# gwall-ceres/HighRes-net

Measured on AMD Instinct MI355X. Metric: SR frames/sec (384x384 out) at B=32, n_views=32, higher is better.
Workload: dtype bf16

## Files before the change

### highres-net_amd/hrnet_hip/csrc/conv3x3_v6_impl.h

```cpp
#pragma once
#include <type_traits>
#include "conv3x3.h"

#ifndef V6_ABL
#define V6_ABL 0
#endif
#ifndef V6_ST_AUX
#define V6_ST_AUX 2
#endif
#ifndef V6_RES_NT
#define V6_RES_NT 1
#endif
#ifndef V6_BAL
#define V6_BAL 4
#endif

#ifdef V6_STAMP
extern __device__ unsigned long long hrn_v6_stamps[256 * 8 * 24];
#define V6_ST(i) do { unsigned long long t_; asm volatile("s_memtime %0\n\ts_waitcnt lgkmcnt(0)" : "=s"(t_) :: "memory"); if (stamp_on) st[i] = t_; } while (0)
#else
#define V6_ST(i) do {} while (0)
#endif

namespace {

constexpr int T6_H = 16, T6_W = 32;
constexpr int HW6 = T6_W + 2;
constexpr int NPIX6 = (T6_H + 2) * HW6;
constexpr int N_IN6 = (NPIX6 * 64 + 1023) / 1024;
constexpr int IN_BYTES6 = N_IN6 * 1024;
constexpr unsigned OOB6 = 0x80000000u;

template <int COUT, bool X3 = false> struct G6 {
    static constexpr int NCB = COUT / 16;
    static constexpr int NQ = NCB / 2;
    static constexpr int TAP_BYTES = COUT * 64;
    static constexpr int WST = 3 * TAP_BYTES;
    static constexpr int W_PIECES = WST / 1024;
    static constexpr int OFF_IN = 2 * WST;
    static constexpr int OFF_BIAS = OFF_IN + 2 * IN_BYTES6;
    static constexpr int ROW = COUT * 2;
    static constexpr int LB = NCB * 2;
    static constexpr int OFF_FIFO = OFF_BIAS + 512;
    static constexpr int FIFO_WAVE = (LB == 16 && !X3) ? 4096 : 0;
    static constexpr int OFF_HOFF = OFF_FIFO + 8 * FIFO_WAVE;
    static constexpr int LDS_BYTES = OFF_HOFF + (X3 ? 8 * 5 * 256 : 0);
};

typedef __attribute__((address_space(3))) void* lds_ptr6;

template <int N> __device__ __forceinline__ void wait_vm6() {
    static_assert(N >= 0 && N <= 63, "vmcnt");
    asm volatile("s_waitcnt vmcnt(%0)" :: "n"(N) : "memory");
}
__device__ __forceinline__ void wait_vm6_rt(int n) {
    switch (n) {
        case 1: wait_vm6<1>(); break;
        case 2: wait_vm6<2>(); break;
        case 3: wait_vm6<3>(); break;
        case 4: wait_vm6<4>(); break;
        case 5: wait_vm6<5>(); break;
        case 6: wait_vm6<6>(); break;
        case 7: wait_vm6<7>(); break;
        case 8: wait_vm6<8>(); break;
        case 9: wait_vm6<9>(); break;
        default: wait_vm6<0>(); break;
    }
}
__device__ __forceinline__ void barrier6() {
    asm volatile("s_waitcnt lgkmcnt(0)" ::: "memory");
    __builtin_amdgcn_s_barrier();
    asm volatile("" ::: "memory");
}
__device__ __forceinline__ int swz6(int row) { return ((row >> 2) & 1) << 1; }

template <int N, int I = 0, class F> __device__ __forceinline__ void static_for6(F&& f) {
    if constexpr (I < N) { f(std::integral_constant<int, I>{}); static_for6<N, I + 1>(f); }
}

template <int CIN, int COUT, int RESM, bool PAIR, bool X3>
__global__ __launch_bounds__(512, 2) void conv3x3_v6_kernel(const ConvParams p) {
    typedef G6<COUT, X3> GEO;
    static_assert(CIN == 128 || (CIN == 64 && !PAIR), "CIN");
    constexpr int NCH = CIN / 32;
    constexpr int NCC = X3 ? 3 * NCH : NCH;
    constexpr int NCB = GEO::NCB, NQ = GEO::NQ, NSTEP = 3 * NQ, WST = GEO::WST, TAP_BYTES = GEO::TAP_BYTES;
    constexpr int OFF_IN = GEO::OFF_IN, ROW = GEO::ROW, LB = GEO::LB;
    typedef typename std::conditional<LB == 16, u32x4, u32x2>::type lane_row_t;
    constexpr bool RES = RESM != 0;
    constexpr int BAL = COUT == 128 ? V6_BAL : 0;
    extern __shared__ __attribute__((aligned(16))) unsigned char smem[];
    float* bias_lds = (float*)(smem + GEO::OFF_BIAS);
    if constexpr (X3) {
        if (p.only_if_nonpos && p.only_if_nonpos[0] > 0.f) return;
    }

    const int tid = threadIdx.x;
    const int lane = tid & 63;
    const int w = __builtin_amdgcn_readfirstlane(tid >> 6);
    const int c15 = lane & 15, q = lane >> 4;
    const int H = p.H, W = p.W;
    const unsigned hw = (unsigned)(H * W);
    const unsigned tiles_x = (W + T6_W - 1) / T6_W;
    const unsigned tiles_y = (H + T6_H - 1) / T6_H;
    const unsigned tiles = tiles_x * tiles_y;
    const unsigned total = tiles * (unsigned)p.M;
    const unsigned G = gridDim.x;
    const unsigned bid = blockIdx.x;
    const unsigned slot0 = (G & 7) == 0 ? (bid & 7) * (G >> 3) + (bid >> 3) : bid;
    if (slot0 >= total) return;
    const int ntl = (int)((total - slot0 + G - 1) / G);
    unsigned cur_m = slot0 / tiles, cur_t = slot0 - cur_m * tiles;
    const unsigned step_m = G / tiles, step_t = G - step_m * tiles;
    constexpr bool in_pair = PAIR;
    constexpr unsigned in_pitch = in_pair ? 128u : (unsigned)(CIN * 2);
    const size_t src_lo = X3 ? (in_pair ? p.stack_lo : p.in_lo) : 0;
    const unsigned char* const src0 = (const unsigned char*)(in_pair ? p.stack : p.in);
    const unsigned img_bytes = hw * in_pitch;

    auto in_bases = [&](unsigned m, size_t& a, size_t& b) __attribute__((always_inline)) {
        if (in_pair) {
            const unsigned bb = m / (unsigned)p.pair_h, i = m - bb * (unsigned)p.pair_h;
            a = ((size_t)bb * p.pair_vs + i) * hw * 128;
            b = ((size_t)bb * p.pair_vs + (p.pair_last - i)) * hw * 128;
        } else {
            a = b = (size_t)m * hw * in_pitch;
        }
    };
    unsigned hoff[5];
    auto tile_offsets = [&](unsigned t) __attribute__((always_inline)) {
        const int ty = t / tiles_x;
        const int y0 = ty * T6_H, x0 = (t - ty * tiles_x) * T6_W;
        int lq = lane;
        asm volatile("" : "+v"(lq));
#pragma unroll
        for (int jj = 0; jj < 5; ++jj) {
            const int pix = (w + 8 * jj) * 16 + (lq >> 2);
            const int lc = (lq & 3) ^ swz6(pix);
            const int py = pix / HW6, px = pix - py * HW6;
            const int gy = y0 - 1 + py, gx = x0 - 1 + px;
            const bool ok = pix < NPIX6 && (unsigned)gy < (unsigned)H && (unsigned)gx < (unsigned)W;
            const unsigned ho = ok ? (unsigned)(gy * W + gx) * in_pitch + (unsigned)(lc * 16) : OOB6;
            if constexpr (X3) *(unsigned*)(smem + GEO::OFF_HOFF + (w * 5 + jj) * 256 + lq * 4) = ho;
            else hoff[jj] = ho;
        }
    };
    auto dma_halo_v = [&](__amdgpu_buffer_rsrc_t rs, int c, int buf, int jj, unsigned voff) __attribute__((always_inline)) {
        const int j = w + 8 * jj;
        if (j < N_IN6) {
            const unsigned soff = in_pair ? (unsigned)((c & 1) * 64) : (unsigned)(c * 64);
            if (!(V6_ABL & 4)) __builtin_amdgcn_raw_ptr_buffer_load_lds(rs, (lds_ptr6)(smem + OFF_IN + buf * IN_BYTES6 + j * 1024), 16, voff, soff, 0, 0);
        }
    };
    auto hoff_lds = [&](int jj) __attribute__((always_inline)) -> unsigned {
        return *(const unsigned*)(smem + GEO::OFF_HOFF + (w * 5 + jj) * 256 + lane * 4);
    };
    auto dma_halo = [&](__amdgpu_buffer_rsrc_t rs, int c, int buf, int jj) __attribute__((always_inline)) {
        if constexpr (X3) dma_halo_v(rs, c, buf, jj, hoff_lds(jj));
        else dma_halo_v(rs, c, buf, jj, hoff[jj]);
    };
    constexpr unsigned W_PLANE = 9u * CIN * COUT * 2u;
    const __amdgpu_buffer_rsrc_t rs_w = __builtin_amdgcn_make_buffer_rsrc((void*)p.wpk, 0, (int)(W_PLANE * (X3 ? 2 : 1)), 0x00020000);
    const unsigned w_lane_off = (unsigned)((lane >> 2) * (NCB * 128) + (((lane & 3) ^ swz6(lane >> 2)) << 4));
    auto dma_w = [&](int c, int tg, int slot_, int t3, unsigned plane_off) __attribute__((always_inline)) {
        const int qq = w + 8 * t3;
        if (qq < GEO::W_PIECES) {
            const int kx = qq / NCB, jb = qq - kx * NCB;
            const unsigned soff = plane_off + (unsigned)(((c >> 1) * 9 + tg * 3 + kx) * (COUT * 128) + (c & 1) * 64 + jb * 128);
            if (!(V6_ABL & 4)) __builtin_amdgcn_raw_ptr_buffer_load_lds(rs_w, (lds_ptr6)(smem + slot_ * WST + kx * TAP_BYTES + jb * 1024), 16, w_lane_off, soff, 0, 0);
        }
    };
    constexpr int NW3 = (GEO::W_PIECES + 7) / 8;
    const int n_in = w < (N_IN6 & 7) ? (N_IN6 >> 3) + 1 : (N_IN6 >> 3);

    const float act_slope = p.slope ? p.slope[0] : 1.f;
    const float act_pick = act_slope <= 1.f ? __builtin_inff() : -__builtin_inff();

    const unsigned lds0 = (unsigned)(__UINTPTR_TYPE__)(__attribute__((address_space(3))) unsigned char*)smem;
    const unsigned a_off = lds0 + (unsigned)(c15 * 64 + ((q ^ swz6(c15)) << 4));
    unsigned baddr[4][3];
#pragma unroll
    for (int j = 0; j < 4; ++j)
#pragma unroll
        for (int kx = 0; kx < 3; ++kx) {
            const int pix = (2 * w + j) * HW6 + c15 + kx;
            baddr[j][kx] = lds0 + (unsigned)OFF_IN + (unsigned)(pix << 6) + ((unsigned)(q << 4) ^ (unsigned)((pix & 4) << 3));
        }

    f32x4 acc[NCB][4];
#ifdef V6_STAMP
    unsigned long long st[24];
#pragma unroll
    for (int i = 0; i < 24; ++i) st[i] = 0;
    bool stamp_on = false;
#endif

    if (tid < COUT) bias_lds[tid] = p.bias[tid];
    size_t inA, inB;
    in_bases(cur_m, inA, inB);
    tile_offsets(cur_t);
    {
        const __amdgpu_buffer_rsrc_t rs = __builtin_amdgcn_make_buffer_rsrc((void*)(src0 + inA), 0, (int)img_bytes, 0x00020000);
#pragma unroll
        for (int t3 = 0; t3 < NW3; ++t3) dma_w(0, 0, 0, t3, 0u);
#pragma unroll
        for (int jj = 0; jj < 5; ++jj) dma_halo(rs, 0, 0, jj);
    }
    wait_vm6<0>();
    barrier6();

    for (int tl = 0; tl < ntl; ++tl) {
        const bool more_tiles = tl + 1 < ntl;
#ifdef V6_STAMP
        stamp_on = false;
        if (RESM == 2 && !PAIR && ntl >= 32 && tl == 1) { stamp_on = true; V6_ST(20); }
        if (RESM == 2 && !PAIR && ntl >= 32 && tl == 2) { stamp_on = true; V6_ST(21); stamp_on = false; }
#endif
        unsigned nxt_t = cur_t + step_t, nxt_m = cur_m + step_m;
        if (nxt_t >= tiles) { nxt_t -= tiles; ++nxt_m; }
        size_t nxA = inA, nxB = inB;
        if (more_tiles) in_bases(nxt_m, nxA, nxB);
#pragma unroll
        for (int cb4 = 0; cb4 < NCB; cb4 += 4) {
            const f32x4 b = *(const f32x4*)(bias_lds + NCB * c15 + cb4);
#pragma unroll
            for (int e = 0; e < 4; ++e)
#pragma unroll
                for (int pxb = 0; pxb < 4; ++pxb) acc[cb4 + e][pxb] = f32x4{b[e], b[e], b[e], b[e]};
        }
        const int ty_ = cur_t / tiles_x;
        const int y0 = ty_ * T6_H, x0 = (cur_t - ty_ * tiles_x) * T6_W;
        const unsigned char *resA = nullptr, *resB = nullptr;
        unsigned char* outp;
        float res_alpha = 1.f;
        {
            size_t oimg = cur_m;
            if (p.out_h > 0) {
                const unsigned ob = cur_m / (unsigned)p.out_h, oi = cur_m - ob * (unsigned)p.out_h;
                oimg = (size_t)ob * p.out_vs + oi;
                if (RESM == 3) {
                    resA = resB = (const unsigned char*)p.res + ((size_t)ob * p.res_vs + oi) * hw * 128;
                    if (p.alphas) res_alpha = p.alphas[(size_t)ob * p.alpha_vs + (p.pair_last - oi)];
                }
            }
            if (RESM == 2) {
                const unsigned bb = cur_m / (unsigned)p.pair_h, i = cur_m - bb * (unsigned)p.pair_h;
                resA = (const unsigned char*)p.stack + ((size_t)bb * p.pair_vs + i) * hw * 128;
                resB = (const unsigned char*)p.stack + ((size_t)bb * p.pair_vs + (p.pair_last - i)) * hw * 128;
            }
            if (RESM == 1) resA = resB = (const unsigned char*)p.res + (size_t)cur_m * hw * ROW;
            outp = (unsigned char*)p.out + oimg * hw * ROW;
        }
        auto res_src = [&](int r, int j) __attribute__((always_inline)) -> const unsigned char* {
            int lq = lane;
            asm volatile("" : "+v"(lq));
            const int c15r = lq & 15, qr = lq >> 4;
            const int gy = y0 + 2 * w + (r >> 1), gyc = gy < H ? gy : H - 1;
            const int gx = x0 + 16 * (r & 1) + 4 * qr + j, gxc = gx < W ? gx : W - 1;
            const unsigned char* view = (RESM == 2 && c15r >= 8) ? resB : resA;
            constexpr int RPITCH = RESM == 1 ? ROW : 128;
            if (V6_ABL & 64) return resA + ((unsigned)(((gyc * W + gxc) & 511) * RPITCH) + (RESM == 2 ? (unsigned)((c15r & 7) * 16) : (unsigned)(c15r * LB)));
            return view + ((unsigned)((gyc * W + gxc) * RPITCH) + (RESM == 2 ? (unsigned)((c15r & 7) * 16) : (unsigned)(c15r * LB)));
        };
        constexpr bool FIFO = RES && LB == 16 && !X3;
        auto res_dma0 = [&]() __attribute__((always_inline)) {
#pragma unroll
            for (int j = 0; j < 4; ++j)
                if (!(V6_ABL & 16))
                    __builtin_amdgcn_global_load_lds((const __attribute__((address_space(1))) void*)res_src(0, j),
                                                     (lds_ptr6)(smem + GEO::OFF_FIFO + w * GEO::FIFO_WAVE + j * 1024), 16, 0, V6_RES_NT ? 2 : 0);
        };

        int c = 0, ps = 0;
        for (int cc = 0; cc < NCC; ++cc) {
            if ((cc > 0 || tl > 0) && (!X3 || ps != 1)) {
                const unsigned d = (X3 ? ps == 2 : (c & 1) != 0) ? (unsigned)IN_BYTES6 : (unsigned)-IN_BYTES6;
#pragma unroll
                for (int j = 0; j < 4; ++j)
#pragma unroll
                    for (int kx = 0; kx < 3; ++kx) baddr[j][kx] += d;
            }
            if (cc == NCC - 1) {
                inA = nxA; inB = nxB;
                if (more_tiles) tile_offsets(nxt_t);
            }
            auto stage = [&](auto tg_c) __attribute__((always_inline)) {
                constexpr int tg = decltype(tg_c)::value;
#ifdef V6_STAMP
                const bool so_ = stamp_on;
                stamp_on = so_ && (cc == 1 || (cc == NCC - 1 && tg == 2));
                const int sb_ = cc == 1 ? 4 * tg : 12;
                V6_ST(sb_ + 0);
#endif
                const int slot_r = (cc + tg) & 1;
                const bool have_next = cc < NCC - 1 || tg < 2 || more_tiles;
                const bool next_chunk = (!X3 || ps != 1) && (cc < NCC - 1 || more_tiles);
                const int tg2 = (tg + 1) % 3;
                int c2 = c;
                unsigned wpl2 = 0;
                if (X3) {
                    int ps2 = ps;
                    if (tg == 2) { if (++ps2 == 3) { ps2 = 0; c2 = (c + 1) & (NCH - 1); } }
                    wpl2 = ps2 == 1 ? W_PLANE : 0u;
                } else {
                    c2 = (c + (tg + 1) / 3) & (NCH - 1);
                }
                const bool nlo = X3 && ps == 0;
                const int cn = nlo ? c : (c + 1) & (NCH - 1);
                const int nbuf = X3 ? (nlo ? 1 : 0) : (cn & 1);
                size_t hb = ((in_pair && cn >= 2) ? inB : inA) + (nlo ? src_lo : (size_t)0);
                if constexpr (X3) {
                    hb = (size_t)(unsigned)__builtin_amdgcn_readfirstlane((int)(unsigned)hb) |
                         ((size_t)(unsigned)__builtin_amdgcn_readfirstlane((int)(unsigned)(hb >> 32)) << 32);
                }
                const __amdgpu_buffer_rsrc_t rs_h = __builtin_amdgcn_make_buffer_rsrc((void*)(src0 + hb), 0, (int)img_bytes, 0x00020000);
                unsigned hst[3] = {0u, 0u, 0u};
                if constexpr (X3) {
                    if (tg < 2 && next_chunk) {
#pragma unroll
                        for (int k = 0; k < (tg == 0 ? 3 : 2); ++k) hst[k] = hoff_lds(tg == 0 ? k : 3 + k);
                        asm volatile("s_waitcnt lgkmcnt(0)" : "+v"(hst[0]), "+v"(hst[1]), "+v"(hst[2]));
                    }
                }
                auto issue_item = [&](int it) __attribute__((always_inline)) {
                    if (it < NW3) { if (have_next) dma_w(c2, tg2, slot_r ^ 1, it, wpl2); }
                    else if (tg == 0 && it < NW3 + 3) {
                        if (next_chunk) { if constexpr (X3) dma_halo_v(rs_h, cn, nbuf, it - NW3, hst[it - NW3]); else dma_halo(rs_h, cn, nbuf, it - NW3); }
                    } else if (tg == 1 && it < NW3 + 2) {
                        if (next_chunk) { if constexpr (X3) dma_halo_v(rs_h, cn, nbuf, it - NW3 + 3, hst[it - NW3]); else dma_halo(rs_h, cn, nbuf, it - NW3 + 3); }
                    }
                };
                constexpr int N_ITEMS = NW3 + (tg == 0 ? 3 : tg == 1 ? 2 : 0);
                static_assert(N_ITEMS <= NSTEP, "one DMA item per step");
                int halo_out = 0;
                if (next_chunk) halo_out = tg == 0 ? 3 : tg == 1 ? n_in - 3 : 0;
                if (FIFO && tg == 2 && cc == NCC - 1 && !(V6_ABL & 2)) res_dma0();
                const unsigned abase = a_off + (unsigned)(slot_r * WST);
                bf16x8 fa[2][2], fb[2][4];
                auto rd = [&](bf16x8& dst, unsigned addr, int imm) __attribute__((always_inline)) {
                    if (V6_ABL & 32) asm volatile("; no read" : "=v"(dst) : "v"(addr), "n"(imm));
                    else asm volatile("ds_read_b128 %0, %1 offset:%2" : "=v"(dst) : "v"(addr), "n"(imm));
                };
                auto load_b1 = [&](int tap, int pxb) __attribute__((always_inline)) {
                    rd(fb[tap & 1][pxb], baddr[(pxb >> 1) + tg][tap], (pxb & 1) * 1024);
                };
                auto load_a1 = [&](int i, int k) __attribute__((always_inline)) {
                    rd(fa[i & 1][k], abase, (i / NQ) * TAP_BYTES + (i % NQ) * 2048 + k * 1024);
                };
                if (BAL && w >= 4) __builtin_amdgcn_s_setprio(1);
#pragma unroll
                for (int pxb = 0; pxb < 4; ++pxb) load_b1(0, pxb);
                load_a1(0, 0);
                load_a1(0, 1);
                __builtin_amdgcn_sched_barrier(0);
                static_for6<NSTEP>([&](auto i_c) __attribute__((always_inline)) {
                    constexpr int i = decltype(i_c)::value;
                    constexpr int qt = i % NQ, tap = i / NQ, bs = tap & 1;
                    constexpr bool a_next = i + 1 < NSTEP;
                    constexpr bool b_cur = qt == (NQ > 1 ? 1 : 0) && tap + 1 < 3;
                    constexpr bool b_prev = i >= 1 && ((i - 1) % NQ) == (NQ > 1 ? 1 : 0) && (i - 1) / NQ + 1 < 3;
                    constexpr int n0 = (b_prev && NQ == 2) ? 0 : 1 + (b_prev ? 4 : 0);
                    constexpr int n4 = (b_prev ? 4 : 0) + (a_next ? 2 : 0) + (b_cur ? 2 : 0);
#pragma unroll
                    for (int g = 0; g < 8; ++g) {
                        const int k = g >> 2, pxb = g & 3;
                        if (g == 0) {
                            if (n0 == 0) asm volatile("s_waitcnt lgkmcnt(0)" : "+v"(fa[i & 1][0]), "+v"(fb[bs][0]), "+v"(fb[bs][1]), "+v"(fb[bs][2]), "+v"(fb[bs][3]));
                            else if (n0 == 1) asm volatile("s_waitcnt lgkmcnt(1)" : "+v"(fa[i & 1][0]), "+v"(fb[bs][0]));
                            else asm volatile("s_waitcnt lgkmcnt(5)" : "+v"(fa[i & 1][0]), "+v"(fb[bs][0]));
                        } else if (g == 4) {
                            if (n4 == 0) asm volatile("s_waitcnt lgkmcnt(0)" : "+v"(fa[i & 1][1]));
                            else if (n4 == 2) asm volatile("s_waitcnt lgkmcnt(2)" : "+v"(fa[i & 1][1]));
                            else if (n4 == 4) asm volatile("s_waitcnt lgkmcnt(4)" : "+v"(fa[i & 1][1]));
                            else if (n4 == 6) asm volatile("s_waitcnt lgkmcnt(6)" : "+v"(fa[i & 1][1]));
                            else asm volatile("s_waitcnt lgkmcnt(8)" : "+v"(fa[i & 1][1]));
                        } else if (k == 0) asm volatile("" : "+v"(fb[bs][pxb]));
                        if (V6_ABL & 1) asm volatile("" : "+v"(acc[qt * 2 + k][pxb]) : "v"(fa[i & 1][k]), "v"(fb[bs][pxb]));
                        else acc[qt * 2 + k][pxb] = __builtin_amdgcn_mfma_f32_16x16x32_bf16(fb[bs][pxb], fa[i & 1][k], acc[qt * 2 + k][pxb], 0, 0, 0);
                        if (g < 2 && a_next) load_a1(i + 1, g);
                        if (g >= 2 && g < 6 && b_cur) load_b1(tap + 1, g - 2);
                        if (g == 7 && i < N_ITEMS) issue_item(i);
                        if (BAL && g == 7 && i == (NSTEP * BAL) / 8 - 1 && w >= 4) __builtin_amdgcn_s_setprio(0);
                        __builtin_amdgcn_sched_barrier(0);
                    }
                });
                V6_ST(sb_ + 1);
                wait_vm6_rt(halo_out);
                V6_ST(sb_ + 2);
                if (tg == 2 && cc == NCC - 1 && (V6_ABL & 2)) {
#pragma unroll
                    for (int cb = 0; cb < NCB; ++cb)
#pragma unroll
                        for (int pxb = 0; pxb < 4; ++pxb) asm volatile("" :: "v"(acc[cb][pxb]));
                }
                if constexpr (X3) {
                if (tg == 2 && cc == NCC - 1 && !(V6_ABL & 2)) {
                    __builtin_amdgcn_s_waitcnt(0x0F70);
                    int le = lane;
                    asm volatile("" : "+v"(le));
                    const int c15e = le & 15, qe = le >> 4;
                    const size_t ob_ = (size_t)outp;
                    unsigned char* const outu = (unsigned char*)((size_t)(unsigned)__builtin_amdgcn_readfirstlane((int)(unsigned)ob_) |
                                                                 ((size_t)(unsigned)__builtin_amdgcn_readfirstlane((int)(unsigned)(ob_ >> 32)) << 32));
                    const __amdgpu_buffer_rsrc_t rs_out = __builtin_amdgcn_make_buffer_rsrc((void*)outu, 0, (int)(hw * ROW), 0x00020000);
                    const __amdgpu_buffer_rsrc_t rs_out_lo = __builtin_amdgcn_make_buffer_rsrc((void*)(outu + p.out_lo), 0, (int)(hw * ROW), 0x00020000);
                    const size_t res_lo_off = RESM == 2 ? p.stack_lo : p.res_lo;
                    lane_row_t rq[8][4];
                    auto res_load = [&](int r, int pl) __attribute__((always_inline)) {
#pragma unroll
                        for (int j = 0; j < 4; ++j)
                            rq[pl * 4 + r][j] = __builtin_nontemporal_load((const lane_row_t*)(res_src(r, j) + (pl ? res_lo_off : (size_t)0)));
                    };
                    if (RES) {
                        res_load(0, 0); res_load(0, 1); res_load(1, 0);
                        if (LB == 8) res_load(1, 1);
                    }
                    __builtin_amdgcn_sched_barrier(0);
#pragma unroll
                    for (int r = 0; r < 4; ++r) {
                        const int gy = y0 + 2 * w + (r >> 1);
#pragma unroll
                        for (int j = 0; j < 4; ++j) {
                            lane_row_t oh, ol;
                            const lane_row_t rh = rq[r][j], rl = rq[4 + r][j];
#pragma unroll
                            for (int i = 0; i < NCB / 2; ++i) {
                                float xa = acc[2 * i][r][j], xb = acc[2 * i + 1][r][j];
                                xa = __builtin_amdgcn_fmed3f(xa, act_slope * xa, act_pick);
                                xb = __builtin_amdgcn_fmed3f(xb, act_slope * xb, act_pick);
                                if (RES) {
                                    const float ra = __uint_as_float(rh[i] << 16), rb = __uint_as_float(rh[i] & 0xffff0000u);
                                    if (RESM == 3) { xa = ra + res_alpha * xa; xb = rb + res_alpha * xb; }
                                    else { xa += ra; xb += rb; }
                                    xa += __uint_as_float(rl[i] << 16); xb += __uint_as_float(rl[i] & 0xffff0000u);
                                }
                                const unsigned h = pack2_bf16(xa, xb);
                                oh[i] = h;
                                ol[i] = pack2_bf16(xa - __uint_as_float(h << 16), xb - __uint_as_float(h & 0xffff0000u));
                            }
                            const int gx = x0 + 16 * (r & 1) + 4 * qe + j;
                            const unsigned voff = (unsigned)((gy * W + gx) * ROW + c15e * LB) | ((unsigned)(W - 1 - gx) & OOB6) | (gy < H ? 0u : OOB6);
                            if constexpr (LB == 16) {
                                __builtin_amdgcn_raw_buffer_store_b128(oh, rs_out, voff, 0, V6_ST_AUX);
                                __builtin_amdgcn_raw_buffer_store_b128(ol, rs_out_lo, voff, 0, V6_ST_AUX);
                            } else {
                                __builtin_amdgcn_raw_buffer_store_b64(oh, rs_out, voff, 0, V6_ST_AUX);
                                __builtin_amdgcn_raw_buffer_store_b64(ol, rs_out_lo, voff, 0, V6_ST_AUX);
                            }
                        }
                        if (RES) {
                            __builtin_amdgcn_sched_barrier(0);
                            if (LB == 16) {
                                if (r == 0) { res_load(1, 1); res_load(2, 0); res_load(2, 1); }
                                if (r == 1) { res_load(3, 0); res_load(3, 1); }
                            } else if (r < 2) { res_load(r + 2, 0); res_load(r + 2, 1); }
                        }
                        __builtin_amdgcn_sched_barrier(0);
                    }
                }
                } else
                if (tg == 2 && cc == NCC - 1 && !(V6_ABL & 2)) {
                    __builtin_amdgcn_s_waitcnt(0x0F70);
                    int le = lane;
                    asm volatile("" : "+v"(le));
                    const int c15e = le & 15, qe = le >> 4;
                    const __amdgpu_buffer_rsrc_t rs_out = __builtin_amdgcn_make_buffer_rsrc((void*)outp, 0, (int)(hw * ROW), 0x00020000);
                    lane_row_t rq[4][4];
                    auto res_load = [&](int r) __attribute__((always_inline)) {
#pragma unroll
                        for (int j = 0; j < 4; ++j) {
                            if (V6_ABL & 16) { rq[r][j] = lane_row_t{}; rq[r][j][0] = (unsigned)le; }
#if V6_RES_NT
                            else rq[r][j] = __builtin_nontemporal_load((const lane_row_t*)res_src(r, j));
#else
                            else rq[r][j] = *(const lane_row_t*)res_src(r, j);
#endif
                        }
                    };
                    if (RES) {
                        if (FIFO) {
                            res_load(1); res_load(2);
#pragma unroll
                            for (int j = 0; j < 4; ++j) rq[0][j] = *(const lane_row_t*)(smem + GEO::OFF_FIFO + w * GEO::FIFO_WAVE + j * 1024 + le * 16);
                        } else { res_load(0); res_load(1); }
                    }
                    __builtin_amdgcn_sched_barrier(0);
                    {
#pragma unroll
                        for (int r = 0; r < 4; ++r) {
                            const int gy = y0 + 2 * w + (r >> 1);
#pragma unroll
                            for (int j = 0; j < 4; ++j) {
                                lane_row_t o;
                                const lane_row_t rv = rq[r][j];
#pragma unroll
                                for (int i = 0; i < NCB / 2; ++i) {
                                    float xa = acc[2 * i][r][j], xb = acc[2 * i + 1][r][j];
                                    xa = __builtin_amdgcn_fmed3f(xa, act_slope * xa, act_pick);
                                    xb = __builtin_amdgcn_fmed3f(xb, act_slope * xb, act_pick);
                                    if (RES) {
                                        const float ra = __uint_as_float(rv[i] << 16), rb = __uint_as_float(rv[i] & 0xffff0000u);
                                        if (RESM == 3) { xa = ra + res_alpha * xa; xb = rb + res_alpha * xb; }
                                        else { xa += ra; xb += rb; }
                                    }
                                    o[i] = pack2_bf16(xa, xb);
                                }
                                const int gx = x0 + 16 * (r & 1) + 4 * qe + j;
                                const unsigned voff = (unsigned)((gy * W + gx) * ROW + c15e * LB) | ((unsigned)(W - 1 - gx) & OOB6) | (gy < H ? 0u : OOB6);
                                if (V6_ABL & 8) asm volatile("" :: "v"(o), "v"(voff));
                                else if constexpr (LB == 16) __builtin_amdgcn_raw_buffer_store_b128(o, rs_out, voff, 0, V6_ST_AUX);
                                else __builtin_amdgcn_raw_buffer_store_b64(o, rs_out, voff, 0, V6_ST_AUX);
                            }
                            if (RES && (FIFO ? r == 0 : r < 2)) res_load(FIFO ? 3 : r + 2);
                            __builtin_amdgcn_sched_barrier(0);
                        }
                    }
                }
#ifdef V6_STAMP
                if (cc == NCC - 1 && tg == 2) V6_ST(16);
#endif
                barrier6();
                V6_ST(sb_ + 3);
#ifdef V6_STAMP
                stamp_on = so_;
#endif
            };
            stage(std::integral_constant<int, 0>{});
            stage(std::integral_constant<int, 1>{});
            stage(std::integral_constant<int, 2>{});
            if (X3) { if (++ps == 3) { ps = 0; ++c; } } else ++c;
        }
        cur_m = nxt_m; cur_t = nxt_t;
    }
    wait_vm6<0>();
#ifdef V6_STAMP
    if (RESM == 2 && !PAIR && ntl >= 32 && lane == 0) {
#pragma unroll
        for (int i = 0; i < 24; ++i) hrn_v6_stamps[(bid * 8 + w) * 24 + i] = st[i];
    }
#endif
}

template <int CIN, int COUT, int RESM, bool PAIR, bool X3>
int launch_v6(const ConvParams& p, long grid, hipStream_t stream) {
    typedef G6<COUT, X3> GEO;
    static_assert(GEO::LDS_BYTES <= 160 * 1024, "LDS budget");
    { const int rc_lds = hrn_allow_lds((const void*)conv3x3_v6_kernel<CIN, COUT, RESM, PAIR, X3>, GEO::LDS_BYTES); if (rc_lds) return rc_lds; }
    hipLaunchKernelGGL((conv3x3_v6_kernel<CIN, COUT, RESM, PAIR, X3>), dim3((unsigned)grid), dim3(512), GEO::LDS_BYTES, stream, p);
    HRN_LAUNCH_CHECK();
    return 0;
}

inline int v6_grid(const ConvParams& p, int cin, long& grid) {
    const long tiles = (long)((p.W + T6_W - 1) / T6_W) * ((p.H + T6_H - 1) / T6_H);
    const long total = tiles * p.M;
    HRN_CHECK(total > 0, -2, "conv3x3_v6: bad tile count %ld", total);
    if (total >= (1L << 30) || (long)p.H * p.W * (cin * 2) >= (1L << 31)) return -100;
    grid = hrn_device_cus();
    if (total < grid) grid = total;
    if (grid >= 8) grid &= ~7L;
    return 0;
}

}
```

Baseline: 2027.

## Stage all nine taps per chunk for COUT=64 conv and prefetch residual into registers

For the COUT=64 non-X3 conv variant, the weight stage now holds all nine 3x3 taps, so each channel chunk runs as a single stage with one barrier instead of three. Halo and weight DMA issue is reworked to fit the single stage. For residual kernels, the residual rows are loaded into registers while the MFMA loop of the last chunk is still running, instead of in the epilogue. This is meant to cut barrier and sync overhead and hide residual-load latency. In exchange it uses more LDS per weight slot and more VGPRs for the residual buffer, which could lower occupancy.

```diff
diff --git a/highres-net_amd/hrnet_hip/csrc/conv3x3_v6_impl.h b/highres-net_amd/hrnet_hip/csrc/conv3x3_v6_impl.h
--- a/highres-net_amd/hrnet_hip/csrc/conv3x3_v6_impl.h
+++ b/highres-net_amd/hrnet_hip/csrc/conv3x3_v6_impl.h
@@ -34,8 +34,9 @@
 template <int COUT, bool X3 = false> struct G6 {
     static constexpr int NCB = COUT / 16;
     static constexpr int NQ = NCB / 2;
+    static constexpr int NT = (COUT == 64 && !X3) ? 9 : 3;
     static constexpr int TAP_BYTES = COUT * 64;
-    static constexpr int WST = 3 * TAP_BYTES;
+    static constexpr int WST = NT * TAP_BYTES;
     static constexpr int W_PIECES = WST / 1024;
     static constexpr int OFF_IN = 2 * WST;
     static constexpr int OFF_BIAS = OFF_IN + 2 * IN_BYTES6;
@@ -84,7 +85,8 @@
     static_assert(CIN == 128 || (CIN == 64 && !PAIR), "CIN");
     constexpr int NCH = CIN / 32;
     constexpr int NCC = X3 ? 3 * NCH : NCH;
-    constexpr int NCB = GEO::NCB, NQ = GEO::NQ, NSTEP = 3 * NQ, WST = GEO::WST, TAP_BYTES = GEO::TAP_BYTES;
+    constexpr int NT = GEO::NT, NSTG = 9 / NT;
+    constexpr int NCB = GEO::NCB, NQ = GEO::NQ, NSTEP = NT * NQ, WST = GEO::WST, TAP_BYTES = GEO::TAP_BYTES;
     constexpr int OFF_IN = GEO::OFF_IN, ROW = GEO::ROW, LB = GEO::LB;
     typedef typename std::conditional<LB == 16, u32x4, u32x2>::type lane_row_t;
     constexpr bool RES = RESM != 0;
@@ -165,9 +167,9 @@
     auto dma_w = [&](int c, int tg, int slot_, int t3, unsigned plane_off) __attribute__((always_inline)) {
         const int qq = w + 8 * t3;
         if (qq < GEO::W_PIECES) {
-            const int kx = qq / NCB, jb = qq - kx * NCB;
-            const unsigned soff = plane_off + (unsigned)(((c >> 1) * 9 + tg * 3 + kx) * (COUT * 128) + (c & 1) * 64 + jb * 128);
-            if (!(V6_ABL & 4)) __builtin_amdgcn_raw_ptr_buffer_load_lds(rs_w, (lds_ptr6)(smem + slot_ * WST + kx * TAP_BYTES + jb * 1024), 16, w_lane_off, soff, 0, 0);
+            const int t = qq / NCB, jb = qq - t * NCB;
+            const unsigned soff = plane_off + (unsigned)(((c >> 1) * 9 + tg * NT + t) * (COUT * 128) + (c & 1) * 64 + jb * 128);
+            if (!(V6_ABL & 4)) __builtin_amdgcn_raw_ptr_buffer_load_lds(rs_w, (lds_ptr6)(smem + slot_ * WST + t * TAP_BYTES + jb * 1024), 16, w_lane_off, soff, 0, 0);
         }
     };
     constexpr int NW3 = (GEO::W_PIECES + 7) / 8;
@@ -293,9 +295,9 @@
                 V6_ST(sb_ + 0);
 #endif
                 const int slot_r = (cc + tg) & 1;
-                const bool have_next = cc < NCC - 1 || tg < 2 || more_tiles;
+                const bool have_next = cc < NCC - 1 || tg < NSTG - 1 || more_tiles;
                 const bool next_chunk = (!X3 || ps != 1) && (cc < NCC - 1 || more_tiles);
-                const int tg2 = (tg + 1) % 3;
+                const int tg2 = (tg + 1) % NSTG;
                 int c2 = c;
                 unsigned wpl2 = 0;
                 if (X3) {
@@ -303,7 +305,7 @@
                     if (tg == 2) { if (++ps2 == 3) { ps2 = 0; c2 = (c + 1) & (NCH - 1); } }
                     wpl2 = ps2 == 1 ? W_PLANE : 0u;
                 } else {
-                    c2 = (c + (tg + 1) / 3) & (NCH - 1);
+                    c2 = (c + (tg + 1) / NSTG) & (NCH - 1);
                 }
                 const bool nlo = X3 && ps == 0;
                 const int cn = nlo ? c : (c + 1) & (NCH - 1);
@@ -323,18 +325,23 @@
                     }
                 }
                 auto issue_item = [&](int it) __attribute__((always_inline)) {
-                    if (it < NW3) { if (have_next) dma_w(c2, tg2, slot_r ^ 1, it, wpl2); }
+                    if constexpr (NT == 9) {
+                        if (it < 5) { if (next_chunk) dma_halo(rs_h, cn, nbuf, it); }
+                        else if (have_next) dma_w(c2, tg2, slot_r ^ 1, it - 5, wpl2);
+                    } else if (it < NW3) { if (have_next) dma_w(c2, tg2, slot_r ^ 1, it, wpl2); }
                     else if (tg == 0 && it < NW3 + 3) {
                         if (next_chunk) { if constexpr (X3) dma_halo_v(rs_h, cn, nbuf, it - NW3, hst[it - NW3]); else dma_halo(rs_h, cn, nbuf, it - NW3); }
                     } else if (tg == 1 && it < NW3 + 2) {
                         if (next_chunk) { if constexpr (X3) dma_halo_v(rs_h, cn, nbuf, it - NW3 + 3, hst[it - NW3]); else dma_halo(rs_h, cn, nbuf, it - NW3 + 3); }
                     }
                 };
-                constexpr int N_ITEMS = NW3 + (tg == 0 ? 3 : tg == 1 ? 2 : 0);
+                constexpr int N_ITEMS = NW3 + (NT == 9 ? 5 : tg == 0 ? 3 : tg == 1 ? 2 : 0);
                 static_assert(N_ITEMS <= NSTEP, "one DMA item per step");
                 int halo_out = 0;
-                if (next_chunk) halo_out = tg == 0 ? 3 : tg == 1 ? n_in - 3 : 0;
-                if (FIFO && tg == 2 && cc == NCC - 1 && !(V6_ABL & 2)) res_dma0();
+                if (NT == 3 && next_chunk) halo_out = tg == 0 ? 3 : tg == 1 ? n_in - 3 : 0;
+                if (FIFO && tg == NSTG - 1 && cc == NCC - 1 && !(V6_ABL & 2)) res_dma0();
+                constexpr bool RES_VREG = RES && NT == 9;
+                lane_row_t rres[4][4];
                 const unsigned abase = a_off + (unsigned)(slot_r * WST);
                 bf16x8 fa[2][2], fb[2][4];
                 auto rd = [&](bf16x8& dst, unsigned addr, int imm) __attribute__((always_inline)) {
@@ -342,7 +349,7 @@
                     else asm volatile("ds_read_b128 %0, %1 offset:%2" : "=v"(dst) : "v"(addr), "n"(imm));
                 };
                 auto load_b1 = [&](int tap, int pxb) __attribute__((always_inline)) {
-                    rd(fb[tap & 1][pxb], baddr[(pxb >> 1) + tg][tap], (pxb & 1) * 1024);
+                    rd(fb[tap & 1][pxb], baddr[(pxb >> 1) + tg + tap / 3][tap % 3], (pxb & 1) * 1024);
                 };
                 auto load_a1 = [&](int i, int k) __attribute__((always_inline)) {
                     rd(fa[i & 1][k], abase, (i / NQ) * TAP_BYTES + (i % NQ) * 2048 + k * 1024);
@@ -357,8 +364,8 @@
                     constexpr int i = decltype(i_c)::value;
                     constexpr int qt = i % NQ, tap = i / NQ, bs = tap & 1;
                     constexpr bool a_next = i + 1 < NSTEP;
-                    constexpr bool b_cur = qt == (NQ > 1 ? 1 : 0) && tap + 1 < 3;
-                    constexpr bool b_prev = i >= 1 && ((i - 1) % NQ) == (NQ > 1 ? 1 : 0) && (i - 1) / NQ + 1 < 3;
+                    constexpr bool b_cur = qt == (NQ > 1 ? 1 : 0) && tap + 1 < NT;
+                    constexpr bool b_prev = i >= 1 && ((i - 1) % NQ) == (NQ > 1 ? 1 : 0) && (i - 1) / NQ + 1 < NT;
                     constexpr int n0 = (b_prev && NQ == 2) ? 0 : 1 + (b_prev ? 4 : 0);
                     constexpr int n4 = (b_prev ? 4 : 0) + (a_next ? 2 : 0) + (b_cur ? 2 : 0);
 #pragma unroll
@@ -379,6 +386,19 @@
                         else acc[qt * 2 + k][pxb] = __builtin_amdgcn_mfma_f32_16x16x32_bf16(fb[bs][pxb], fa[i & 1][k], acc[qt * 2 + k][pxb], 0, 0, 0);
                         if (g < 2 && a_next) load_a1(i + 1, g);
                         if (g >= 2 && g < 6 && b_cur) load_b1(tap + 1, g - 2);
+                        if constexpr (RES_VREG && i < 4) {
+                            if (g == 3 && cc == NCC - 1 && !(V6_ABL & 2)) {
+#pragma unroll
+                                for (int j = 0; j < 4; ++j) {
+                                    if (V6_ABL & 16) rres[i][j] = lane_row_t{};
+#if V6_RES_NT
+                                    else rres[i][j] = __builtin_nontemporal_load((const lane_row_t*)res_src(i, j));
+#else
+                                    else rres[i][j] = *(const lane_row_t*)res_src(i, j);
+#endif
+                                }
+                            }
+                        }
                         if (g == 7 && i < N_ITEMS) issue_item(i);
                         if (BAL && g == 7 && i == (NSTEP * BAL) / 8 - 1 && w >= 4) __builtin_amdgcn_s_setprio(0);
                         __builtin_amdgcn_sched_barrier(0);
@@ -387,14 +407,14 @@
                 V6_ST(sb_ + 1);
                 wait_vm6_rt(halo_out);
                 V6_ST(sb_ + 2);
-                if (tg == 2 && cc == NCC - 1 && (V6_ABL & 2)) {
+                if (tg == NSTG - 1 && cc == NCC - 1 && (V6_ABL & 2)) {
 #pragma unroll
                     for (int cb = 0; cb < NCB; ++cb)
 #pragma unroll
                         for (int pxb = 0; pxb < 4; ++pxb) asm volatile("" :: "v"(acc[cb][pxb]));
                 }
                 if constexpr (X3) {
-                if (tg == 2 && cc == NCC - 1 && !(V6_ABL & 2)) {
+                if (tg == NSTG - 1 && cc == NCC - 1 && !(V6_ABL & 2)) {
                     __builtin_amdgcn_s_waitcnt(0x0F70);
                     int le = lane;
                     asm volatile("" : "+v"(le));
@@ -459,7 +479,7 @@
                     }
                 }
                 } else
-                if (tg == 2 && cc == NCC - 1 && !(V6_ABL & 2)) {
+                if (tg == NSTG - 1 && cc == NCC - 1 && !(V6_ABL & 2)) {
                     __builtin_amdgcn_s_waitcnt(0x0F70);
                     int le = lane;
                     asm volatile("" : "+v"(le));
@@ -478,7 +498,12 @@
                         }
                     };
                     if (RES) {
-                        if (FIFO) {
+                        if (RES_VREG) {
+#pragma unroll
+                            for (int r = 0; r < 4; ++r)
+#pragma unroll
+                                for (int j = 0; j < 4; ++j) rq[r][j] = rres[r][j];
+                        } else if (FIFO) {
                             res_load(1); res_load(2);
 #pragma unroll
                             for (int j = 0; j < 4; ++j) rq[0][j] = *(const lane_row_t*)(smem + GEO::OFF_FIFO + w * GEO::FIFO_WAVE + j * 1024 + le * 16);
@@ -511,7 +536,7 @@
                                 else if constexpr (LB == 16) __builtin_amdgcn_raw_buffer_store_b128(o, rs_out, voff, 0, V6_ST_AUX);
                                 else __builtin_amdgcn_raw_buffer_store_b64(o, rs_out, voff, 0, V6_ST_AUX);
                             }
-                            if (RES && (FIFO ? r == 0 : r < 2)) res_load(FIFO ? 3 : r + 2);
+                            if (RES && !RES_VREG && (FIFO ? r == 0 : r < 2)) res_load(FIFO ? 3 : r + 2);
                             __builtin_amdgcn_sched_barrier(0);
                         }
                     }
@@ -526,8 +551,10 @@
 #endif
             };
             stage(std::integral_constant<int, 0>{});
-            stage(std::integral_constant<int, 1>{});
-            stage(std::integral_constant<int, 2>{});
+            if constexpr (NSTG == 3) {
+                stage(std::integral_constant<int, 1>{});
+                stage(std::integral_constant<int, 2>{});
+            }
             if (X3) { if (++ps == 3) { ps = 0; ++c; } } else ++c;
         }
         cur_m = nxt_m; cur_t = nxt_t;
```

After: 2030, median of 6. About the same (+0.1%).
